# alexranaldi/CWSL_DIGI

Measured on AMD Instinct MI355X. Metric: IQ Msamples/s demod+sync per GPU; concurrent FT8 slots at real-time; % HBM roofline, higher is better.
Workload: dtype f32

## Files before the change

### cwsl_digi_amd/csrc/sync_kernels.hpp

```cpp
#pragma once
#include <hip/hip_runtime.h>
#include <stdint.h>

namespace cwslg {

constexpr int FT8_NSPS = 1920, FT8_NSTEP = 480, FT8_NHSYM = 372, FT8_NH1 = 1920, FT8_JZ = 62, FT8_NMAX = 180000;
constexpr int FT4_NFFT1 = 2304, FT4_NSTEP = 576, FT4_NHSYM = 122, FT4_NH1 = 1152, FT4_NMAX = 72576;
constexpr int FT4_ROW = 1168;
constexpr int SYNC_BAND = 32;
constexpr int SYNC_MAXCAND_CAP = 600;
constexpr int SYNC_MAXPRE = 1000;

struct SyncConfig {
    bool enabled = false;
    float syncmin = 1.5f;
    float syncmin_ft4 = 1.2f;
    int max_cand = 200;
    int f_lo_hz = 200, f_hi_hz = 3000;
    int ia = 64, ib = 960, nbins = 976;
    struct Kept {
        bool ft4_coherent = true;
        int order = 0;
        bool ft4_soft = false;
        bool ft8_soft = false;
// ... 973 lines not shown
            for (int k = 0; k < 7; ++k) {
                const float2 v = *reinterpret_cast<const float2 *>(&s_s[rr + 2 * k][2 * mp]);
                acc.x = acc.x + v.x;
                acc.y = acc.y + v.y;
            }
            *reinterpret_cast<float2 *>(c0 + 2 * mp) = acc;
        }
        __builtin_amdgcn_fence(__ATOMIC_RELEASE, "wavefront");
        __builtin_amdgcn_wave_barrier();
        __builtin_amdgcn_fence(__ATOMIC_ACQUIRE, "wavefront");
        const int j = 2 * lane - FT8_JZ;
        const bool ok0 = j <= FT8_JZ, ok1 = j + 1 <= FT8_JZ;
        SyncPair sy = SyncPair{0.0f, 0.0f};
        if (ok0) sy = costas_sync2(s_s, c0, rr, j);
        const unsigned long long ka = ok0 ? sync_key(sy.a, j + FT8_JZ) : 0ull;
        const unsigned long long kb = ok1 ? sync_key(sy.b, j + 1 + FT8_JZ) : 0ull;
        unsigned long long k2 = (kb > ka) ? kb : ka;
        unsigned long long k1 = 0ull;
        if (ok0 && j >= -10 && j <= 10) k1 = ka;
        if (ok1 && j + 1 >= -10 && j + 1 <= 10 && kb > k1) k1 = kb;
        k2 = wave_max_u64(k2);
        k1 = wave_max_u64(k1);
        if (lane == 0) {
            w->red[bin] = key_value(k1);  w->jpeak[bin] = (255 - (int)(k1 & 0xFFu)) - FT8_JZ;
            w->red2[bin] = key_value(k2); w->jpeak2[bin] = (255 - (int)(k2 & 0xFFu)) - FT8_JZ;
        }
        __builtin_amdgcn_fence(__ATOMIC_RELEASE, "wavefront");
        __builtin_amdgcn_wave_barrier();
    }
}

#endif
constexpr int S2_PITCH = 378, S2_COL0 = 2;
constexpr int DPP_ROW_MIRROR = 0x140;

__device__ __forceinline__ float wave_max_f32(float v)
{
    v = fmaxf(v, dpp_get<DPP_XOR1>(v));
    v = fmaxf(v, dpp_get<DPP_XOR2>(v));
    v = fmaxf(v, dpp_get<DPP_HALF_MIRROR>(v));
    v = fmaxf(v, dpp_get<DPP_ROW_MIRROR>(v));
    const int vi = __float_as_int(v);
    const float r0 = __int_as_float(__builtin_amdgcn_readlane(vi, 0)), r1 = __int_as_float(__builtin_amdgcn_readlane(vi, 16));
    const float r2 = __int_as_float(__builtin_amdgcn_readlane(vi, 32)), r3 = __int_as_float(__builtin_amdgcn_readlane(vi, 48));
    return fmaxf(fmaxf(r0, r1), fmaxf(r2, r3));
}

__device__ __forceinline__ void wave_first_max(float v, int lag, float &best, int &best_lag)
{
    const float m = wave_max_f32(v);
    const unsigned long long hit = __builtin_amdgcn_ballot_w64(v == m);
    const int src = hit ? (int)__builtin_ctzll(hit) : 0;
    best = __int_as_float(__builtin_amdgcn_readlane(__float_as_int(v), src));
    best_lag = __builtin_amdgcn_readlane(lag, src);
}

#ifndef CWSLG_SEARCH_HOISTPTR
#define CWSLG_SEARCH_HOISTPTR 1
#endif
#ifndef CWSLG_SEARCH_DPPMAX
#define CWSLG_SEARCH_DPPMAX 1
#endif
__device__ __forceinline__ void wave_first_max2(float va, int laga, float vb, int lagb, float &besta, int &best_laga, float &bestb, int &best_lagb)
{
    float ma = va, mb = vb;
#define CWSLG_DPP_MAX2(CTRL)                                                                  \
    "v_max_f32_dpp %0, %0, %0 " CTRL "\n\t"                                                   \
    "v_max_f32_dpp %1, %1, %1 " CTRL "\n\t"                                                   \
    "s_nop 0\n\t"
    asm volatile("s_nop 1\n\t"
                 CWSLG_DPP_MAX2("quad_perm:[1,0,3,2] row_mask:0xf bank_mask:0xf")
                 CWSLG_DPP_MAX2("quad_perm:[2,3,0,1] row_mask:0xf bank_mask:0xf")
                 CWSLG_DPP_MAX2("row_half_mirror row_mask:0xf bank_mask:0xf")
                 CWSLG_DPP_MAX2("row_mirror row_mask:0xf bank_mask:0xf")
                 CWSLG_DPP_MAX2("row_bcast:15 row_mask:0xa bank_mask:0xf")
                 CWSLG_DPP_MAX2("row_bcast:31 row_mask:0xc bank_mask:0xf")
                 "s_nop 0"
                 : "+v"(ma), "+v"(mb));
#undef CWSLG_DPP_MAX2
    const float wa = __int_as_float(__builtin_amdgcn_readlane(__float_as_int(ma), 63));
    const float wb = __int_as_float(__builtin_amdgcn_readlane(__float_as_int(mb), 63));
    const unsigned long long hita = __builtin_amdgcn_ballot_w64(va == wa), hitb = __builtin_amdgcn_ballot_w64(vb == wb);
    const int srca = hita ? (int)__builtin_ctzll(hita) : 0, srcb = hitb ? (int)__builtin_ctzll(hitb) : 0;
    besta = __int_as_float(__builtin_amdgcn_readlane(__float_as_int(va), srca)); best_laga = __builtin_amdgcn_readlane(laga, srca);
    bestb = __int_as_float(__builtin_amdgcn_readlane(__float_as_int(vb), srcb)); best_lagb = __builtin_amdgcn_readlane(lagb, srcb);
}

__device__ __forceinline__ float div6_exact(float x)
{
    const float r = 0x1.555556p-3f;
    const float q0 = x * r;
    const float e = __builtin_fmaf(-6.0f, q0, x);
    float q = __builtin_fmaf(e, r, q0);
    if (__builtin_expect((__float_as_uint(x) & 0x7fffffffu) - 0x10000000u >= 0x6f800000u, 0)) q = x / 6.0f;
    return q;
}

__device__ __forceinline__ float sync_finish(float ta, float tb, float tc, float t0a, float t0b, float t0c)
{
    float t = ta + tb + tc;
    float t0 = t0a + t0b + t0c;
    t0 = div6_exact(t0 - t);
    const float sync_abc = t / t0;
    t = tb + tc;
    t0 = t0b + t0c;
    t0 = div6_exact(t0 - t);
    const float sync_bc = t / t0;
    float sy = (sync_abc > sync_bc) ? sync_abc : sync_bc;
    if (!(sy == sy)) sy = 0.0f;
    return sy;
}

__device__ __forceinline__ void sync_finish2(v2f ta, v2f tb, v2f tc, v2f ua, v2f ub, v2f uc, float &sx, float &sy)
{
    const float r = 0x1.555556p-3f;
    const float t1x = ta.x + tb.x + tc.x, t1y = ta.y + tb.y + tc.y;
    const float d1x = (ua.x + ub.x + uc.x) - t1x, d1y = (ua.y + ub.y + uc.y) - t1y;
    const float t2x = tb.x + tc.x, t2y = tb.y + tc.y;
    const float d2x = (ub.x + uc.x) - t2x, d2y = (ub.y + uc.y) - t2y;
    auto short6 = [&](float x) { const float q0 = x * r; return __builtin_fmaf(__builtin_fmaf(-6.0f, q0, x), r, q0); };
    auto biased = [](float x) { return (__float_as_uint(x) & 0x7fffffffu) - 0x10000000u; };
    float q1x = short6(d1x), q1y = short6(d1y), q2x = short6(d2x), q2y = short6(d2y);
    const unsigned worst = max(max(biased(d1x), biased(d1y)), max(biased(d2x), biased(d2y)));
    if (__builtin_expect(worst >= 0x6f800000u, 0)) { q1x = d1x / 6.0f; q1y = d1y / 6.0f; q2x = d2x / 6.0f; q2y = d2y / 6.0f; }
    const float ax = t1x / q1x, bx = t2x / q2x, ay = t1y / q1y, by = t2y / q2y;
    sx = (ax > bx) ? ax : bx;
    sy = (ay > by) ? ay : by;
    if (!(sx == sx)) sx = 0.0f;
    if (!(sy == sy)) sy = 0.0f;
}

#if defined(CWSLG_STAMP) && defined(CWSLG_STAMP_SYNC)
#define SSTAMP(slot)                                                                                \
    do {                                                                                            \
        const unsigned wg_ = blockIdx.y * gridDim.x + blockIdx.x;                                   \
        if (threadIdx.x == 0 && wg_ < 65536) {                                                      \
            unsigned long long t_;                                                                  \
            asm volatile("s_waitcnt vmcnt(0) lgkmcnt(0)\n\ts_memtime %0\n\ts_waitcnt lgkmcnt(0)" : "=s"(t_)::"memory");              \
            g_stamps[8 * wg_ + (slot)] = t_;                                                        \
        }                                                                                           \
    } while (0)
#define SSTAMP1(slot)                                                                               \
    do {                                                                                            \
        const unsigned wg_ = blockIdx.y * gridDim.x + blockIdx.x;                                   \
        if (threadIdx.x == 0 && wg_ < 65536) {                                                      \
            unsigned long long t_;                                                                  \
            asm volatile("s_waitcnt lgkmcnt(0)\n\ts_memtime %0\n\ts_waitcnt lgkmcnt(0)" : "=s"(t_)::"memory");              \
            g_stamps[8 * wg_ + (slot)] = t_;                                                        \
        }                                                                                           \
    } while (0)
#else
#define SSTAMP(slot) do { } while (0)
#define SSTAMP1(slot) do { } while (0)
#endif
#if CWSLG_LAB
__global__ __launch_bounds__(SYNC2D_NT, 4) void ft8_sync2d_v2_kernel(const SyncWork *__restrict__ works, int ia, int ib, int nbins)
{
    constexpr int ROWS = SYNC_BAND + 12, NW = SYNC2D_NT / 64;
    constexpr int UN = (FT8_NHSYM + NW - 1) / NW;
    __shared__ __attribute__((aligned(16))) float s_s[ROWS][S2_PITCH];
    __shared__ __attribute__((aligned(16))) float s_c0[NW][S2_PITCH];
    const SyncWork *w = works + blockIdx.y;
    const int tid = threadIdx.x, lane = tid & 63, wv = tid >> 6;
    const int i0 = ia + blockIdx.x * SYNC_BAND;
    {
        const CWSLG_GLOBAL float *sp = as_global(w->spectra) + i0 + lane;
        const bool on = lane < ROWS && i0 + lane < nbins;
        float v[UN];
#pragma unroll
        for (int q = 0; q < UN; ++q) {
            const int m = wv + NW * q;
            v[q] = (on && m < FT8_NHSYM) ? sp[(size_t)m * nbins] : 0.0f;
        }
        float *dst = &s_s[lane < ROWS ? lane : 0][S2_COL0 + 1 + wv];
#pragma unroll
        for (int q = 0; q < UN; ++q)
            if (lane < ROWS && wv + NW * q < FT8_NHSYM) dst[NW * q] = v[q];
        if (tid < ROWS) {
            float *row = s_s[tid];
            row[0] = 0.0f; row[1] = 0.0f; row[2] = 0.0f;
            row[S2_COL0 + 373] = 0.0f; row[S2_COL0 + 374] = 0.0f; row[S2_COL0 + 375] = 0.0f;
        }
    }
    __syncthreads();
    float *c0 = s_c0[wv];
    const int icos[7] = {3, 1, 4, 0, 6, 5, 2};
    const int j = 2 * lane - FT8_JZ;
    const bool ok0 = j <= FT8_JZ, ok1 = j + 1 <= FT8_JZ;
    const bool near0 = j >= -10 && j <= 10, near1 = j + 1 >= -10 && j + 1 <= 10;
    const float ninf = -__builtin_huge_valf();
    const int pa0 = lane - 24, pb0 = pa0 + 72, pc0 = pa0 + 144;
    constexpr int PP = S2_PITCH / 2;
    const v2f *s_s2 = reinterpret_cast<const v2f *>(&s_s[0][0]);
    v2f *c02 = reinterpret_cast<v2f *>(c0);
    {
        for (int rr = wv; rr < SYNC_BAND; rr += NW) {
            const int bin = i0 + rr;
            if (bin > ib) break;
            for (int mp = lane; mp < PP; mp += 64) {
                v2f acc = {0.0f, 0.0f};
#pragma unroll
                for (int k = 0; k < 7; ++k) acc = acc + s_s2[(rr + 2 * k) * PP + mp];
                c02[mp] = acc;
            }
            __builtin_amdgcn_fence(__ATOMIC_RELEASE, "wavefront");
            __builtin_amdgcn_wave_barrier();
            __builtin_amdgcn_fence(__ATOMIC_ACQUIRE, "wavefront");
            v2f ta = {0, 0}, tb = {0, 0}, tc = {0, 0}, ua = {0, 0}, ub = {0, 0}, uc = {0, 0};
#pragma unroll
            for (int n = 0; n < 7; ++n) {
                const v2f *row = s_s2 + (rr + 2 * icos[n]) * PP;
                int pa = pa0 + 2 * n; pa = pa < 0 ? 0 : pa;
                int pc = pc0 + 2 * n; pc = pc > PP - 1 ? PP - 1 : pc;
                const int pb = pb0 + 2 * n;
                const v2f va = row[pa], wa = c02[pa];
                const v2f vb = row[pb], wb = c02[pb];
                const v2f vc = row[pc], wc = c02[pc];
                ta = ta + va; ua = ua + wa;
                tb = tb + vb; ub = ub + wb;
                tc = tc + vc; uc = uc + wc;
            }
            const float sa = ok0 ? sync_finish(ta.x, tb.x, tc.x, ua.x, ub.x, uc.x) : ninf;
            const float sb = ok1 ? sync_finish(ta.y, tb.y, tc.y, ua.y, ub.y, uc.y) : ninf;
            const bool b2 = sb > sa;
            float r2; int l2;
            wave_first_max(b2 ? sb : sa, b2 ? j + 1 : j, r2, l2);
            const float na = near0 ? sa : ninf, nb = near1 ? sb : ninf;
            const bool b1 = nb > na;
            float r1; int l1;
            wave_first_max(b1 ? nb : na, b1 ? j + 1 : j, r1, l1);
            if (lane == 0) {
                as_global_rw(w->red)[bin] = r1;  as_global_rw(w->jpeak)[bin] = l1;
                as_global_rw(w->red2)[bin] = r2; as_global_rw(w->jpeak2)[bin] = l2;
            }
            __builtin_amdgcn_fence(__ATOMIC_RELEASE, "wavefront");
            __builtin_amdgcn_wave_barrier();
        }
    }
}

#endif
#include "sync2d_asm.inc"
template <int NW>
__device__ __forceinline__ void sync2d_search_band(const SyncWork *w, unsigned s_base, unsigned sC, int wvu, int lane, int i0, int ia, int ib)
{
    constexpr int PP = S2_PITCH / 2, RB = S2_PITCH * 4;
    static_assert(S2_PITCH == 378, "sync2d_asm.inc is generated for this row pitch");
    const int j = 2 * lane - FT8_JZ;
    const bool ok0 = j <= FT8_JZ, ok1 = j + 1 <= FT8_JZ;
    const bool near0 = j >= -10 && j <= 10, near1 = j + 1 >= -10 && j + 1 <= 10;
    const float ninf = -__builtin_huge_valf();
    unsigned vA[7], vC[3];
#pragma unroll
    for (int n = 0; n < 7; ++n) { const int p = lane - 24 + 2 * n; vA[n] = 8u * (unsigned)(p < 0 ? 0 : p); }
#pragma unroll
    for (int n = 4; n < 7; ++n) { const int p = lane + 120 + 2 * n; vC[n - 4] = 8u * (unsigned)(p > PP - 1 ? PP - 1 : p); }
    const unsigned vU = 8u * (unsigned)lane, vL2 = 8u * (unsigned)(lane + 128 > PP - 1 ? PP - 1 : lane + 128);
#if CWSLG_SEARCH_HOISTPTR
    float *const p_red = w->red, *const p_red2 = w->red2;
    int *const p_jpeak = w->jpeak, *const p_jpeak2 = w->jpeak2;
#endif
    int rr = wvu;
    while (rr < SYNC_BAND && i0 + rr < ia) rr += NW;
    bool live = rr < SYNC_BAND && i0 + rr <= ib;
    if (live) {
        const unsigned sN = (unsigned)__builtin_amdgcn_readfirstlane((int)(s_base + (unsigned)rr * RB));
        asm volatile(SYNC2D_ASM_C0_ONLY : : [vU] "v"(vU), [vL2] "v"(vL2), [sC] "s"(sC), [sN] "s"(sN) : SYNC2D_ASM_CLOBBERS);
    }
    SSTAMP(2);
    const int rr0 = rr;
    while (live) {
        const int bin = i0 + rr;
        const int rn = rr + NW;
        const bool more = rn < SYNC_BAND && i0 + rn <= ib;
        const unsigned sS = (unsigned)__builtin_amdgcn_readfirstlane((int)(s_base + (unsigned)rr * RB));
        const unsigned sN = sS + NW * RB;
        v2f ta, tb, tc, ua, ub, uc;
        if (more)
            asm volatile(SYNC2D_ASM_SEARCH_NEXT
                         : [ta] "=&v"(ta), [ua] "=&v"(ua), [tb] "=&v"(tb), [ub] "=&v"(ub), [tc] "=&v"(tc), [uc] "=&v"(uc)
                         : [vA0] "v"(vA[0]), [vA1] "v"(vA[1]), [vA2] "v"(vA[2]), [vA3] "v"(vA[3]), [vA4] "v"(vA[4]), [vA5] "v"(vA[5]), [vA6] "v"(vA[6]),
                           [vC4] "v"(vC[0]), [vC5] "v"(vC[1]), [vC6] "v"(vC[2]), [vU] "v"(vU), [vL2] "v"(vL2), [sS] "s"(sS), [sC] "s"(sC), [sN] "s"(sN)
                         : SYNC2D_ASM_CLOBBERS);
        else
            asm volatile(SYNC2D_ASM_SEARCH_LAST
                         : [ta] "=&v"(ta), [ua] "=&v"(ua), [tb] "=&v"(tb), [ub] "=&v"(ub), [tc] "=&v"(tc), [uc] "=&v"(uc)
                         : [vA0] "v"(vA[0]), [vA1] "v"(vA[1]), [vA2] "v"(vA[2]), [vA3] "v"(vA[3]), [vA4] "v"(vA[4]), [vA5] "v"(vA[5]), [vA6] "v"(vA[6]),
                           [vC4] "v"(vC[0]), [vC5] "v"(vC[1]), [vC6] "v"(vC[2]), [vU] "v"(vU), [sS] "s"(sS), [sC] "s"(sC)
                         : SYNC2D_ASM_CLOBBERS);
        if (rr == rr0) SSTAMP(3);
        float sa, sb;
#if CWSLG_SEARCH_DPPMAX
        sync_finish2(ta, tb, tc, ua, ub, uc, sa, sb);
#else
        sa = sync_finish(ta.x, tb.x, tc.x, ua.x, ub.x, uc.x);
        sb = sync_finish(ta.y, tb.y, tc.y, ua.y, ub.y, uc.y);
#endif
        asm volatile("" : "+v"(sa), "+v"(sb));
        sa = ok0 ? sa : ninf;
        sb = ok1 ? sb : ninf;
        if (rr == rr0) SSTAMP(4);
        const bool b2 = sb > sa;
        const float na = near0 ? sa : ninf, nb = near1 ? sb : ninf;
        const bool b1 = nb > na;
        float r1, r2; int l1, l2;
#if CWSLG_SEARCH_DPPMAX
        wave_first_max2(b2 ? sb : sa, b2 ? j + 1 : j, b1 ? nb : na, b1 ? j + 1 : j, r2, l2, r1, l1);
#else
        wave_first_max(b2 ? sb : sa, b2 ? j + 1 : j, r2, l2);
        wave_first_max(b1 ? nb : na, b1 ? j + 1 : j, r1, l1);
#endif
        if (lane == 0) {
#if CWSLG_SEARCH_HOISTPTR
            as_global_rw(p_red)[bin] = r1;  as_global_rw(p_jpeak)[bin] = l1;
            as_global_rw(p_red2)[bin] = r2; as_global_rw(p_jpeak2)[bin] = l2;
#else
            as_global_rw(w->red)[bin] = r1;  as_global_rw(w->jpeak)[bin] = l1;
            as_global_rw(w->red2)[bin] = r2; as_global_rw(w->jpeak2)[bin] = l2;
#endif
        }
        if (rr == rr0) SSTAMP(5);
        rr = rn;
        live = more;
    }
}

__global__ __launch_bounds__(SYNC2D_NT, 4) void ft8_sync2d_v3_kernel(const SyncWork *__restrict__ works, int ia, int ib, int nbins)
{
    constexpr int ROWS = SYNC_BAND + 12, NW = SYNC2D_NT / 64;
    constexpr int UN = (FT8_NHSYM + NW - 1) / NW;
    __shared__ __attribute__((aligned(16))) float s_s[ROWS][S2_PITCH];
    __shared__ __attribute__((aligned(16))) float s_c0[NW][S2_PITCH];
    const SyncWork *w = works + blockIdx.y;
    const int tid = threadIdx.x, lane = tid & 63, wv = tid >> 6;
    const int i0 = ia + blockIdx.x * SYNC_BAND;
    SSTAMP(0);
    {
        const CWSLG_GLOBAL float *sp = as_global(w->spectra) + i0 + lane;
        const bool on = lane < ROWS && i0 + lane < nbins;
        float v[UN];
#pragma unroll
        for (int q = 0; q < UN; ++q) {
            const int m = wv + NW * q;
            v[q] = (on && m < FT8_NHSYM) ? plane_load1(sp + (size_t)m * nbins) : 0.0f;
        }
        float *dst = &s_s[lane < ROWS ? lane : 0][S2_COL0 + 1 + wv];
#pragma unroll
        for (int q = 0; q < UN; ++q)
            if (lane < ROWS && wv + NW * q < FT8_NHSYM) dst[NW * q] = v[q];
        if (tid < ROWS) {
            float *row = s_s[tid];
            row[0] = 0.0f; row[1] = 0.0f; row[2] = 0.0f;
            row[S2_COL0 + 373] = 0.0f; row[S2_COL0 + 374] = 0.0f; row[S2_COL0 + 375] = 0.0f;
        }
    }
    __syncthreads();
    SSTAMP(1);
    const int wvu = __builtin_amdgcn_readfirstlane(wv);
    const unsigned s_base = (unsigned)(uintptr_t)&s_s[0][0];
    const unsigned sC = (unsigned)__builtin_amdgcn_readfirstlane((int)((unsigned)(uintptr_t)&s_c0[0][0] + (unsigned)wvu * (S2_PITCH * 4)));
#ifdef CWSLG_SYNC_STAGGER
    if (wvu >= NW / 2) __builtin_amdgcn_s_sleep(CWSLG_SYNC_STAGGER);
#endif
    sync2d_search_band<NW>(w, s_base, sC, wvu, lane, i0, ia, ib);
    SSTAMP(6);
}

__device__ __forceinline__ bool key_less(float va, int ia_, float vb, int ib_)
{
    if (va < vb) return true;
    if (va > vb) return false;
    return ia_ < ib_;
}

template <int NT>
__device__ void bitonic_sort_n(float *kv, int *ki, int n, int tid)
{
    for (int size = 2; size <= n; size <<= 1) {
        for (int stride = size >> 1; stride >= 1; stride >>= 1) {
            for (int t = tid; t < n / 2; t += NT) {
                const int lo = 2 * t - (t & (stride - 1));
                const int hi = lo + stride;
                const bool up = (lo & size) == 0;
                const float a = kv[lo], b = kv[hi];
                const int ai = ki[lo], bi = ki[hi];
                const bool sw = up ? key_less(b, bi, a, ai) : key_less(a, ai, b, bi);
                if (sw) { kv[lo] = b; kv[hi] = a; ki[lo] = bi; ki[hi] = ai; }
            }
            __syncthreads();
        }
    }
}

template <int NT>
struct CandLds {
    static constexpr size_t kv = 0, ki = kv + 2048 * 4, red = ki + 2048 * 4, red2 = red + (FT8_NH1 + 1) * 4 + 12, jp = red2 + (FT8_NH1 + 1) * 4 + 12,
                            jp2 = jp + (FT8_NH1 + 1) * 2 + 14, first = jp2 + (FT8_NH1 + 1) * 2 + 14, second = first + (FT8_NH1 + 2) * 2 + 12,
                            desc = second + (FT8_NH1 + 2) * 2 + 12, scan = desc + SYNC_MAXPRE * 4, scan_lo = scan + NT * 4, cbin = scan_lo + 1024 * 4,
                            clag = cbin + SYNC_MAXPRE * 4, csync = clag + SYNC_MAXPRE * 4, cf = csync + SYNC_MAXPRE * 4, ct = cf + SYNC_MAXPRE * 4,
                            base = ct + SYNC_MAXPRE * 4, n = base + 16, bytes = n + 16;
};

template <int NT>
__device__ void ft8_candidates_body(const SyncWork *w, int ia, int ib, float syncmin, int maxcand, int order, char *lds)
{
    using L = CandLds<NT>;
    float *s_kv = reinterpret_cast<float *>(lds + L::kv);
    int *s_ki = reinterpret_cast<int *>(lds + L::ki);
    float *s_red = reinterpret_cast<float *>(lds + L::red), *s_red2 = reinterpret_cast<float *>(lds + L::red2);
    short *s_jp = reinterpret_cast<short *>(lds + L::jp), *s_jp2 = reinterpret_cast<short *>(lds + L::jp2);
    short *s_first = reinterpret_cast<short *>(lds + L::first), *s_second = reinterpret_cast<short *>(lds + L::second);
    int *s_desc = reinterpret_cast<int *>(lds + L::desc);
    int *s_scan = reinterpret_cast<int *>(lds + L::scan);
    unsigned *s_scan_lo = reinterpret_cast<unsigned *>(lds + L::scan_lo);
    int *s_cbin = reinterpret_cast<int *>(lds + L::cbin), *s_clag = reinterpret_cast<int *>(lds + L::clag);
    float *s_csync = reinterpret_cast<float *>(lds + L::csync), *s_cf = reinterpret_cast<float *>(lds + L::cf), *s_ct = reinterpret_cast<float *>(lds + L::ct);
    float *s_base = reinterpret_cast<float *>(lds + L::base);
    int &s_n = *reinterpret_cast<int *>(lds + L::n);
    const int tid = threadIdx.x;
    const int iz = ib - ia + 1;
    const float df = 12000.0f / 3840.0f, tstep = 480.0f / 12000.0f;
    for (int i = ia + tid; i <= ib; i += NT) {
        s_red[i] = as_global(w->red)[i]; s_red2[i] = as_global(w->red2)[i]; s_jp[i] = (short)as_global(w->jpeak)[i]; s_jp2[i] = (short)as_global(w->jpeak2)[i];
    }
    for (int i = tid; i < FT8_NH1 + 2; i += NT) { s_first[i] = -1; s_second[i] = -1; }
    const int npct = (int)lroundf(0.40f * (float)iz);
    const int lim = min(SYNC_MAXPRE, iz);
    const int nsort = (iz <= 1024) ? 1024 : 2048;
    __syncthreads();
    for (int k = tid; k < nsort; k += NT) { s_kv[k] = (k < iz) ? s_red2[ia + k] : __builtin_huge_valf(); s_ki[k] = (k < iz) ? ia + k : 0x7fffffff; }
    __syncthreads();
    bitonic_sort_n<NT>(s_kv, s_ki, nsort, tid);
    if (tid == 0 && npct >= 1) s_base[1] = s_red2[s_ki[npct - 1]];
    __syncthreads();
    for (int k = tid; k < nsort; k += NT) { s_kv[k] = (k < iz) ? s_red[ia + k] : __builtin_huge_valf(); s_ki[k] = (k < iz) ? ia + k : 0x7fffffff; }
    __syncthreads();
    bitonic_sort_n<NT>(s_kv, s_ki, nsort, tid);
    if (tid == 0 && npct >= 1) s_base[0] = s_red[s_ki[npct - 1]];
    for (int r = tid; r < lim; r += NT) s_desc[r] = s_ki[iz - 1 - r];
    __syncthreads();
    if (npct < 1) { if (tid == 0) *as_global_rw(w->ncand) = 0; return; }
    const float base = s_base[0], base2 = s_base[1];
    for (int i = ia + tid; i <= ib; i += NT) { s_red[i] = s_red[i] / base; s_red2[i] = s_red2[i] / base2; }
    __syncthreads();
    constexpr int PER = (SYNC_MAXPRE + NT - 1) / NT;
    int cnt[PER], flags[PER];
    int local = 0;
#pragma unroll
    for (int q = 0; q < PER; ++q) {
        const int r = tid * PER + q;
        int f = 0;
        if (r < lim) {
            const int n = s_desc[r];
            if (s_red[n] >= syncmin) f |= 1;
            if (s_jp2[n] != s_jp[n] && s_red2[n] >= syncmin) f |= 2;
        }
        flags[q] = f;
        cnt[q] = (f & 1) + ((f >> 1) & 1);
        local += cnt[q];
    }
    s_scan[tid] = local;
    __syncthreads();
    for (int off = 1; off < NT; off <<= 1) {
        const int v = (tid >= off) ? s_scan[tid - off] : 0;
        __syncthreads();
        s_scan[tid] += v;
        __syncthreads();
    }
    int pos = s_scan[tid] - local;
#pragma unroll
    for (int q = 0; q < PER; ++q) {
        const int r = tid * PER + q;
        if (r < lim) {
            const int n = s_desc[r];
            if ((flags[q] & 1) && pos < SYNC_MAXPRE) { s_cbin[pos] = n; s_clag[pos] = s_jp[n]; s_csync[pos] = s_red[n]; s_first[n] = (short)pos; }
            if (flags[q] & 1) ++pos;
            if ((flags[q] & 2) && pos < SYNC_MAXPRE) { s_cbin[pos] = n; s_clag[pos] = s_jp2[n]; s_csync[pos] = s_red2[n]; s_second[n] = (short)pos; }
            if (flags[q] & 2) ++pos;
        }
    }
    if (tid == NT - 1) s_n = min(s_scan[NT - 1], SYNC_MAXPRE);
    __syncthreads();
    const int ncand = s_n;
    for (int i = tid; i < ncand; i += NT) { s_cf[i] = (float)s_cbin[i] * df; s_ct[i] = ((float)s_clag[i] - 0.5f) * tstep; }
    __syncthreads();
    short *s_done = reinterpret_cast<short *>(s_ki);
    short *s_ready = s_done + SYNC_MAXPRE;
    for (int i = tid; i < ncand; i += NT) s_done[i] = 0;
    __syncthreads();
    for (int round = 0; round <= ncand; ++round) {
        int pending = 0;
        for (int i = tid; i < ncand; i += NT) {
            if (s_done[i]) { s_ready[i] = 0; continue; }
            const int n = s_cbin[i];
            bool ok = true;
#pragma unroll
            for (int dn = -2; dn <= 2; ++dn) {
                const int nb = n + dn;
                if (nb < 0 || nb > FT8_NH1) continue;
                const int a = s_first[nb], b = s_second[nb];
                if (a >= 0 && a < i && !s_done[a]) ok = false;
                if (b >= 0 && b < i && !s_done[b]) ok = false;
            }
            s_ready[i] = ok ? 1 : 0;
            pending = 1;
        }
        if (!__syncthreads_or(pending)) break;
        for (int i = tid; i < ncand; i += NT) {
            if (!s_ready[i]) continue;
            const int n = s_cbin[i];
            int part[6];
            int np = 0;
#pragma unroll
            for (int dn = -1; dn <= 1; ++dn) {
                const int nb = n + dn;
                if (nb < 0 || nb > FT8_NH1) continue;
                const int a = s_first[nb], b = s_second[nb];
                if (a >= 0 && a < i) part[np++] = a;
                if (b >= 0 && b < i) part[np++] = b;
            }
#pragma unroll
            for (int x = 1; x < 6; ++x) {
                if (x < np) {
                    const int v = part[x];
                    int y = x - 1;
                    while (y >= 0 && part[y] > v) { part[y + 1] = part[y]; --y; }
                    part[y + 1] = v;
                }
            }
            const float fi = fabsf(s_cf[i]), ti = s_ct[i];
            float si = s_csync[i];
            for (int x = 0; x < np; ++x) {
                const int j = part[x];
                const float fdiff = fi - fabsf(s_cf[j]);
                const float tdiff = fabsf(ti - s_ct[j]);
                if (fabsf(fdiff) < 4.0f && tdiff < 0.04f) {
                    const float sj = s_csync[j];
                    if (si >= sj) s_csync[j] = 0.0f;
                    if (si < sj) si = 0.0f;
                }
            }
            s_csync[i] = si;
            s_done[i] = 1;
        }
        __syncthreads();
    }
    __syncthreads();
    unsigned *s_hi = reinterpret_cast<unsigned *>(s_kv);
    unsigned *s_lo = reinterpret_cast<unsigned *>(s_scan_lo);
    for (int i = tid; i < 1024; i += NT) {
        unsigned hi = 0xFFFFFFFFu, lo = 0xFFFFFFFFu;
        if (i < ncand && s_csync[i] >= syncmin) {
            unsigned u = __float_as_uint(s_csync[i]);
            u = (u & 0x80000000u) ? ~u : (u | 0x80000000u);
            hi = ~u;
            lo = ((unsigned)s_cbin[i] << 20) | ((unsigned)(s_clag[i] + FT8_JZ) << 12) | (unsigned)i;
            if (order) { hi = (unsigned)s_cbin[i]; lo = (unsigned)i; }
        }
        s_hi[i] = hi; s_lo[i] = lo;
    }
    __syncthreads();
    for (int size = 2; size <= 1024; size <<= 1) {
        for (int stride = size >> 1; stride >= 1; stride >>= 1) {
            for (int t = tid; t < 512; t += NT) {
                const int l0 = 2 * t - (t & (stride - 1));
                const int h0 = l0 + stride;
                const bool up = (l0 & size) == 0;
                const unsigned long long ka = ((unsigned long long)s_hi[l0] << 32) | s_lo[l0];
                const unsigned long long kb = ((unsigned long long)s_hi[h0] << 32) | s_lo[h0];
                const bool sw = up ? (kb < ka) : (ka < kb);
                if (sw) { s_hi[l0] = (unsigned)(kb >> 32); s_lo[l0] = (unsigned)kb; s_hi[h0] = (unsigned)(ka >> 32); s_lo[h0] = (unsigned)ka; }
            }
            __syncthreads();
        }
    }
    int nout = 0;
    for (int r = tid; r < 1024; r += NT) {
        if (s_hi[r] == 0xFFFFFFFFu && s_lo[r] == 0xFFFFFFFFu) continue;
        ++nout;
        if (r < maxcand) {
            const int i = (int)(s_lo[r] & 0xFFFu);
            CWSLG_GLOBAL SyncChannelBuffers::Cand *c = as_global_rw(w->cand) + r;
            c->freq_bin = s_cbin[i]; c->time_step = s_clag[i]; c->sync = s_csync[i]; c->freq_hz = s_cf[i]; c->dt_s = s_ct[i];
        }
    }
    if (tid == 0) s_n = 0;
    __syncthreads();
    if (nout) atomicAdd(&s_n, nout);
    __syncthreads();
    if (tid == 0) *as_global_rw(w->ncand) = min(s_n, maxcand);
}

template <int NT>
__global__ __launch_bounds__(NT) void ft8_candidates_kernel(const SyncWork *__restrict__ works, int ia, int ib,
                                                              float syncmin, int maxcand, int order)
{
    __shared__ __attribute__((aligned(16))) char s_pool[CandLds<NT>::bytes];
    ft8_candidates_body<NT>(works + blockIdx.x, ia, ib, syncmin, maxcand, order, s_pool);
}

constexpr int SYNCC_NT = 512;
__global__ __launch_bounds__(SYNCC_NT, 4) void ft8_sync_chan_kernel(const SyncWork *__restrict__ works, int ia, int ib, int nbins,
                                                                     float syncmin, int maxcand, int order)
{
    constexpr int ROWS = SYNC_BAND + 12, NW = SYNCC_NT / 64;
    constexpr int UN = (FT8_NHSYM + NW - 1) / NW;
    constexpr int PF = (FT8_NHSYM + 8 * NW - 1) / (8 * NW);
    constexpr size_t IMG_BYTES = (size_t)(ROWS + NW) * S2_PITCH * sizeof(float);
    constexpr size_t POOL_BYTES = IMG_BYTES > CandLds<SYNCC_NT>::bytes ? IMG_BYTES : CandLds<SYNCC_NT>::bytes;
    __shared__ __attribute__((aligned(16))) char s_pool[POOL_BYTES];
    float (*s_s)[S2_PITCH] = reinterpret_cast<float (*)[S2_PITCH]>(s_pool);
    float (*s_c0)[S2_PITCH] = reinterpret_cast<float (*)[S2_PITCH]>(s_pool + (size_t)ROWS * S2_PITCH * sizeof(float));
    const SyncWork *w = works + blockIdx.x;
    const int tid = threadIdx.x, lane = tid & 63, wv = tid >> 6;
    const int i_first = ia - (((ia - 20) % 32) + 32) % 32;
    const int nbands = (ib - i_first) / SYNC_BAND + 1;
    const CWSLG_GLOBAL float *spec = as_global(w->spectra);
    {
        const int col = i_first + lane;
        const bool on = lane < ROWS && col >= 0 && col < nbins;
        const CWSLG_GLOBAL float *sp = spec + (on ? col : 0);
        float v[UN];
#pragma unroll
        for (int q = 0; q < UN; ++q) {
            const int m = wv + NW * q;
            v[q] = (on && m < FT8_NHSYM) ? plane_load1(sp + (size_t)m * nbins) : 0.0f;
        }
        float *dst = &s_s[lane < ROWS ? lane : 0][S2_COL0 + 1 + wv];
#pragma unroll
        for (int q = 0; q < UN; ++q)
            if (lane < ROWS && wv + NW * q < FT8_NHSYM) dst[NW * q] = v[q];
        if (tid < ROWS) {
            float *row = s_s[tid];
            row[0] = 0.0f; row[1] = 0.0f; row[2] = 0.0f;
            row[S2_COL0 + 373] = 0.0f; row[S2_COL0 + 374] = 0.0f; row[S2_COL0 + 375] = 0.0f;
        }
    }
    __syncthreads();
    const int wvu = __builtin_amdgcn_readfirstlane(wv);
    const unsigned s_base = (unsigned)(uintptr_t)&s_s[0][0];
    const unsigned sC = (unsigned)__builtin_amdgcn_readfirstlane((int)((unsigned)(uintptr_t)&s_c0[0][0] + (unsigned)wvu * (S2_PITCH * 4)));
    const int s8 = lane >> 3, g4 = 4 * (lane & 7);
    for (int band = 0; band < nbands; ++band) {
        const int i0 = i_first + band * SYNC_BAND;
        v4f pf[PF];
        const bool more = band + 1 < nbands;
        if (band == 1) SSTAMP(0);
        if (more) {
            const int col = i0 + ROWS + g4;
            const bool on = col < nbins;
            const unsigned o0 = (unsigned)((on ? col : 0) + (8 * wv + s8) * nbins);
            const unsigned ostep = (unsigned)(8 * NW * nbins);
#pragma unroll
            for (int q = 0; q < PF; ++q) {
                const int m = 8 * (wv + NW * q) + s8;
                pf[q] = (on && m < FT8_NHSYM) ? plane_load4(reinterpret_cast<const CWSLG_GLOBAL v4f *>(spec + o0 + (unsigned)q * ostep)) : v4f{0.f, 0.f, 0.f, 0.f};
            }
        }
        if (band == 1) SSTAMP1(1);
        sync2d_search_band<NW>(w, s_base, sC, wvu, lane, i0, ia, ib);
        if (band == 1) SSTAMP1(6);
        if (!more) break;
        constexpr int NMV = 12 * S2_PITCH / 4, MVT = (NMV + SYNCC_NT - 1) / SYNCC_NT;
        static_assert((12 * S2_PITCH) % 4 == 0 && (SYNC_BAND * S2_PITCH) % 4 == 0, "16-byte moves");
        v4f mv[MVT];
#pragma unroll
        for (int q = 0; q < MVT; ++q) {
            const int e = tid + SYNCC_NT * q;
            mv[q] = (e < NMV) ? reinterpret_cast<const v4f *>(&s_s[SYNC_BAND][0])[e] : v4f{0.f, 0.f, 0.f, 0.f};
        }
        __syncthreads();
#pragma unroll
        for (int q = 0; q < MVT; ++q) {
            const int e = tid + SYNCC_NT * q;
            if (e < NMV) reinterpret_cast<v4f *>(&s_s[0][0])[e] = mv[q];
        }
        {
#pragma unroll
            for (int q = 0; q < PF; ++q) {
                const int m = 8 * (wv + NW * q) + s8;
                if (m < FT8_NHSYM) {
#pragma unroll
                    for (int e = 0; e < 4; ++e) s_s[12 + g4 + e][S2_COL0 + 1 + m] = pf[q][e];
                }
            }
        }
        __syncthreads();
        if (band == 1) SSTAMP(7);
    }
    __syncthreads();
    ft8_candidates_body<SYNCC_NT>(w, ia, ib, syncmin, maxcand, order, s_pool);
}

__device__ __forceinline__ double log10_fixed(double x)
{
    if (!(x > 0.0)) return -1.0e300;
    int e = 0;
    double m = x;
    while (m >= 1.4142135623730951) { m = m * 0.5; ++e; }
    while (m < 0.7071067811865476) { m = m * 2.0; --e; }
    const double t = (m - 1.0) / (m + 1.0), t2 = t * t;
    double s = 0.0;
    for (int k = 21; k >= 1; k -= 2) s = s * t2 + 1.0 / (double)k;
    const double ln_m = 2.0 * t * s;
    return ((double)e * 0.6931471805599453 + ln_m) * 0.4342944819032518;
}
__device__ __forceinline__ double exp10_fixed(double y)
{
    const double z = y * 3.321928094887362;
    double fl = (double)(long long)z;
    if (fl > z) fl = fl - 1.0;
    const double f = (z - fl) * 0.6931471805599453;
    double s = 1.0;
    for (int k = 22; k >= 1; --k) s = 1.0 + s * f / (double)k;
    long long n = (long long)fl;
    double p = 1.0;
    if (n >= 0) { for (long long q = 0; q < n && q < 2000; ++q) p = p * 2.0; }
    else { for (long long q = 0; q < -n && q < 2000; ++q) p = p * 0.5; }
    return s * p;
}

__global__ __launch_bounds__(256) void ft4_candidates_kernel(const SyncWork *__restrict__ works, int nfa, int nfb,
                                                              float syncmin, int maxcand, int order)
{
    constexpr int NB1 = FT4_NH1 + 1;
    __shared__ float s_savg[NB1], s_savsm[NB1], s_sdb[NB1], s_sbase[NB1];
    __shared__ float s_segbase[10];
    __shared__ double s_a[5];
    __shared__ double s_A[5][6];
    __shared__ int s_scan[256];
    __shared__ int s_ok;
    __shared__ int s_cbin[SYNC_MAXCAND_CAP];
    __shared__ float s_cs[SYNC_MAXCAND_CAP], s_cf[SYNC_MAXCAND_CAP];
    __shared__ unsigned s_hi[1024], s_lo[1024];
    const SyncWork *w = works + blockIdx.x;
    const int tid = threadIdx.x;
    const CWSLG_GLOBAL float *sp = as_global(w->spectra);
    CWSLG_GLOBAL int *ncand_out = as_global_rw(w->ncand);
    const float df = 12000.0f / (float)FT4_NFFT1;
    for (int i = tid; i < NB1; i += 256) {
        float acc = 0.0f;
        if (i >= 1) {
            for (int j = 0; j < FT4_NHSYM; ++j) acc = acc + sp[(size_t)j * FT4_ROW + i];
            acc = acc / (float)FT4_NHSYM;
        }
        s_savg[i] = acc; s_sbase[i] = 0.0f; s_sdb[i] = 0.0f;
    }
    if (tid == 0) s_ok = 1;
    __syncthreads();
    for (int i = tid; i < NB1; i += 256) {
        float t = 0.0f;
        if (i >= 8 && i <= FT4_NH1 - 7) {
#pragma unroll
            for (int q = -7; q <= 7; ++q) t = t + s_savg[i + q];
            t = t / 15.0f;
        }
        s_savsm[i] = t;
    }
    const int ia = nfa, ib = min(nfb, FT4_NH1);
    const int nseg = 10;
    const int nlen = (ib - ia + 1) / nseg, i0 = (ib - ia + 1) / 2;
    const double half = (double)(ib - ia + 1) / 2.0;
    const bool range_ok = (nfb - nfa) >= 20;
    if (!range_ok) { if (tid == 0) *ncand_out = 0; return; }
    for (int i = ia + tid; i <= ib; i += 256) s_sdb[i] = (float)(10.0 * log10_fixed((double)s_savg[i]));
    __syncthreads();
    {
        int jp = (int)lroundf(((float)nlen * 0.01f) * 10.0f);
        if (jp < 1) jp = 1;
        if (jp > nlen) jp = nlen;
        for (int e = tid; e < nseg * nlen; e += 256) {
            const int seg = e / nlen, q = e - seg * nlen;
            const int ja = ia + seg * nlen;
            const float v = s_sdb[ja + q];
            int less = 0, eq = 0;
            for (int x = 0; x < nlen; ++x) {
                const float o = s_sdb[ja + x];
                less += (o < v) ? 1 : 0;
                eq += (o == v) ? 1 : 0;
            }
            if (less <= jp - 1 && jp - 1 < less + eq) s_segbase[seg] = v;
        }
    }
    __syncthreads();
    if (tid == 0) {
        double S[9], Tm[5];
        for (int q = 0; q < 9; ++q) S[q] = 0.0;
        for (int q = 0; q < 5; ++q) Tm[q] = 0.0;
        int kz = 0;
        for (int n = 0; n < nseg; ++n) {
            const int ja = ia + n * nlen, jb = ja + nlen - 1;
            const float base = s_segbase[n];
            for (int i = ja; i <= jb; ++i) {
                if (s_sdb[i] <= base && kz < 1000) {
                    ++kz;
                    const double u = (double)(i - i0) / half, y = (double)s_sdb[i];
                    double p = 1.0;
                    for (int q = 0; q < 9; ++q) { S[q] = S[q] + p; if (q < 5) Tm[q] = Tm[q] + y * p; p = p * u; }
                }
            }
        }
        int ok = kz >= 5;
        double (&A)[5][6] = s_A;
        for (int r = 0; r < 5; ++r) { for (int cc = 0; cc < 5; ++cc) A[r][cc] = S[r + cc]; A[r][5] = Tm[r]; }
        for (int col = 0; col < 5 && ok; ++col) {
            int piv = col;
            for (int r = col + 1; r < 5; ++r) if (fabs(A[r][col]) > fabs(A[piv][col])) piv = r;
            if (A[piv][col] == 0.0) { ok = 0; break; }
            if (piv != col) for (int cc = 0; cc < 6; ++cc) { const double t = A[col][cc]; A[col][cc] = A[piv][cc]; A[piv][cc] = t; }
            for (int r = col + 1; r < 5; ++r) {
                const double f = A[r][col] / A[col][col];
                for (int cc = col; cc < 6; ++cc) A[r][cc] = A[r][cc] - f * A[col][cc];
            }
        }
        double a[5] = {0, 0, 0, 0, 0};
        if (ok) {
            for (int r = 4; r >= 0; --r) {
                double t = A[r][5];
                for (int cc = r + 1; cc < 5; ++cc) t = t - A[r][cc] * a[cc];
                a[r] = t / A[r][r];
            }
        }
        for (int q = 0; q < 5; ++q) s_a[q] = a[q];
        s_ok = ok;
    }
    __syncthreads();
    if (!s_ok) { if (tid == 0) *ncand_out = 0; return; }
    int bad = 0;
    for (int i = ia + tid; i <= ib; i += 256) {
        const double u = (double)(i - i0) / half;
        const float db = (float)(s_a[0] + u * (s_a[1] + u * (s_a[2] + u * (s_a[3] + u * s_a[4]))) + 0.65);
        const float b = (float)exp10_fixed((double)db / 10.0);
        s_sbase[i] = b;
        if (!(b > 0.0f)) bad = 1;
    }
    if (__syncthreads_or(bad)) { if (tid == 0) *ncand_out = 0; return; }
    for (int i = nfa + tid; i <= nfb; i += 256) s_savsm[i] = s_savsm[i] / s_sbase[i];
    __syncthreads();
    {
        CWSLG_GLOBAL float *red = as_global_rw(w->red), *red2 = as_global_rw(w->red2);
        for (int i = tid; i < NB1; i += 256) { red[i] = s_savsm[i]; red2[i] = s_sbase[i]; }
// ... 81 lines not shown
```

Measured before the change: 302,200.

## Sort candidates in registers with DPP lane exchanges and wave-level scan

Replaces the LDS-based bitonic sorts (two red/red2 percentile sorts and the final candidate sort) with a register-resident bitonic network. Compares within a lane run in registers, cross-lane strides use DPP/permlane swaps, and only large strides go through double-buffered LDS with a barrier. The block-wide Hillis-Steele prefix scan becomes a DPP wave scan plus a per-wave combine. Together these cut the many __syncthreads and LDS round trips in candidate selection. The cost is higher register pressure, more template instantiation, and a final sort sized to the next power of two of the candidate count. Optional timestamp hooks are also added for profiling.

Result: no change. 303,900 (median of 6 runs) (+0.6%).

```diff
diff --git a/cwsl_digi_amd/csrc/sync_kernels.hpp b/cwsl_digi_amd/csrc/sync_kernels.hpp
--- a/cwsl_digi_amd/csrc/sync_kernels.hpp
+++ b/cwsl_digi_amd/csrc/sync_kernels.hpp
@@ -1149,6 +1149,15 @@
 #else
 #define SSTAMP(slot) do { } while (0)
 #define SSTAMP1(slot) do { } while (0)
+#endif
+#if defined(CWSLG_STAMP) && defined(CWSLG_STAMP_SYNC) && defined(CWSLG_STAMP_SEL)
+#define SELSTAMP(slot) SSTAMP(slot)
+#define BANDSTAMP(slot) do { } while (0)
+#define BANDSTAMP1(slot) do { } while (0)
+#else
+#define SELSTAMP(slot) do { } while (0)
+#define BANDSTAMP(slot) SSTAMP(slot)
+#define BANDSTAMP1(slot) SSTAMP1(slot)
 #endif
 #if CWSLG_LAB
 __global__ __launch_bounds__(SYNC2D_NT, 4) void ft8_sync2d_v2_kernel(const SyncWork *__restrict__ works, int ia, int ib, int nbins)
@@ -1370,23 +1379,102 @@
     return ia_ < ib_;
 }
 
-template <int NT>
-__device__ void bitonic_sort_n(float *kv, int *ki, int n, int tid)
-{
-    for (int size = 2; size <= n; size <<= 1) {
-        for (int stride = size >> 1; stride >= 1; stride >>= 1) {
-            for (int t = tid; t < n / 2; t += NT) {
-                const int lo = 2 * t - (t & (stride - 1));
-                const int hi = lo + stride;
-                const bool up = (lo & size) == 0;
-                const float a = kv[lo], b = kv[hi];
-                const int ai = ki[lo], bi = ki[hi];
-                const bool sw = up ? key_less(b, bi, a, ai) : key_less(a, ai, b, bi);
-                if (sw) { kv[lo] = b; kv[hi] = a; ki[lo] = bi; ki[hi] = ai; }
-            }
+struct SortKey { unsigned a, b; };
+struct FloatIndexLess {
+    static __device__ __forceinline__ bool either(SortKey p, SortKey k, bool first)
+    {
+        const float pv = __uint_as_float(p.a), kv = __uint_as_float(k.a);
+        const bool less_pk = (pv < kv) | (((int)p.b < (int)k.b) & !(pv > kv));
+        return less_pk == first;
+    }
+};
+struct WordPairLess {
+    static __device__ __forceinline__ bool either(SortKey p, SortKey k, bool first)
+    {
+        const unsigned long long pk = ((unsigned long long)p.a << 32) | p.b, kk = ((unsigned long long)k.a << 32) | k.b;
+        return (pk < kk) == first;
+    }
+};
+struct SortBufs {
+    char *base;
+    unsigned off0, off1;
+    int flip;
+};
+template <int M>
+__device__ __forceinline__ unsigned lane_xor(unsigned v)
+{
+    static_assert(M == 1 || M == 2 || M == 4 || M == 8 || M == 16 || M == 32, "one bit of the lane number");
+    if constexpr (M == 1) return (unsigned)__builtin_amdgcn_update_dpp((int)v, (int)v, 0xB1, 0xf, 0xf, false);
+    else if constexpr (M == 2) return (unsigned)__builtin_amdgcn_update_dpp((int)v, (int)v, 0x4E, 0xf, 0xf, false);
+    else if constexpr (M == 8) return (unsigned)__builtin_amdgcn_update_dpp((int)v, (int)v, 0x128, 0xf, 0xf, false);
+    else if constexpr (M == 4) {
+        const int t = __builtin_amdgcn_update_dpp((int)v, (int)v, 0x104, 0xf, 0x5, false);
+        return (unsigned)__builtin_amdgcn_update_dpp(t, (int)v, 0x114, 0xf, 0xa, false);
+    } else if constexpr (M == 16) {
+        const auto s = __builtin_amdgcn_permlane16_swap(v, v, false, false);
+        return (__lane_id() & 16) ? s[0] : s[1];
+    } else {
+        const auto s = __builtin_amdgcn_permlane32_swap(v, v, false, false);
+        return (__lane_id() & 32) ? s[0] : s[1];
+    }
+}
+template <class LESS, int NT, int K, int SIZE, int STRIDE>
+__device__ __forceinline__ void sort_stage(SortKey (&k)[K], int tid, SortBufs &sb)
+{
+    if constexpr (STRIDE < K) {
+#pragma unroll
+        for (int r = 0; r < K; ++r) {
+            if (r & STRIDE) continue;
+            const bool up = ((tid * K + r) & SIZE) == 0;
+            const SortKey a = k[r], b = k[r + STRIDE];
+            const bool sw = LESS::either(b, a, up);
+            k[r].a = sw ? b.a : a.a; k[r].b = sw ? b.b : a.b;
+            k[r + STRIDE].a = sw ? a.a : b.a; k[r + STRIDE].b = sw ? a.b : b.b;
+        }
+    } else {
+        SortKey p[K];
+        if constexpr (STRIDE / K < 64) {
+#pragma unroll
+            for (int r = 0; r < K; ++r) { p[r].a = lane_xor<STRIDE / K>(k[r].a); p[r].b = lane_xor<STRIDE / K>(k[r].b); }
+        } else {
+            unsigned *pa = reinterpret_cast<unsigned *>(sb.base + (sb.flip ? sb.off1 : sb.off0)), *pb = pa + NT * K;
+            sb.flip ^= 1;
+#pragma unroll
+            for (int r = 0; r < K; ++r) { pa[tid * K + r] = k[r].a; pb[tid * K + r] = k[r].b; }
             __syncthreads();
-        }
-    }
+            const int j = (tid * K) ^ STRIDE;
+#pragma unroll
+            for (int r = 0; r < K; ++r) { p[r].a = pa[j + r]; p[r].b = pb[j + r]; }
+        }
+        const bool is_hi = ((tid * K) & STRIDE) != 0, up = ((tid * K) & SIZE) == 0;
+        const bool first = up != is_hi;
+#pragma unroll
+        for (int r = 0; r < K; ++r) {
+            const bool sw = LESS::either(p[r], k[r], first);
+            k[r].a = sw ? p[r].a : k[r].a; k[r].b = sw ? p[r].b : k[r].b;
+        }
+    }
+}
+template <class LESS, int NT, int K, int SIZE, int STRIDE>
+__device__ __forceinline__ void sort_strides(SortKey (&k)[K], int tid, SortBufs &sb)
+{
+    sort_stage<LESS, NT, K, SIZE, STRIDE>(k, tid, sb);
+    if constexpr (STRIDE > 1) sort_strides<LESS, NT, K, SIZE, STRIDE / 2>(k, tid, sb);
+}
+template <class LESS, int NT, int K, int SIZE = 2>
+__device__ __forceinline__ void sort_in_registers(SortKey (&k)[K], int n, int tid, SortBufs &sb)
+{
+    if (SIZE <= n) sort_strides<LESS, NT, K, SIZE, SIZE / 2>(k, tid, sb);
+    if constexpr (SIZE < NT * K) sort_in_registers<LESS, NT, K, 2 * SIZE>(k, n, tid, sb);
+}
+__device__ __forceinline__ int wave_scan_add(int x, int lane)
+{
+    x += __builtin_amdgcn_update_dpp(0, x, 0x111, 0xf, 0xf, false);
+    x += __builtin_amdgcn_update_dpp(0, x, 0x112, 0xf, 0xf, false);
+    x += __builtin_amdgcn_update_dpp(0, x, 0x114, 0xf, 0xf, false);
+    x += __builtin_amdgcn_update_dpp(0, x, 0x118, 0xf, 0xf, false);
+    const int r0 = __builtin_amdgcn_readlane(x, 15), r1 = __builtin_amdgcn_readlane(x, 31), r2 = __builtin_amdgcn_readlane(x, 47);
+    return x + (lane >= 16 ? r0 : 0) + (lane >= 32 ? r1 : 0) + (lane >= 48 ? r2 : 0);
 }
 
 template <int NT>
@@ -1398,18 +1486,45 @@
                             base = ct + SYNC_MAXPRE * 4, n = base + 16, bytes = n + 16;
 };
 
+template <int NT, int K>
+__device__ __forceinline__ void red_orders(char *lds, int ia, int iz, int npct, int lim, int tid)
+{
+    using L = CandLds<NT>;
+    static_assert(NT * K <= 2048 && 2 * (size_t)NT * K * 4 <= L::red - L::kv && 2 * (size_t)NT * K * 4 <= L::base - L::cbin, "the sorts' two LDS buffers");
+    int *s_desc = reinterpret_cast<int *>(lds + L::desc);
+    float *s_base = reinterpret_cast<float *>(lds + L::base);
+    SortBufs sb{lds, (unsigned)L::kv, (unsigned)L::cbin, 0};
+#pragma unroll 1
+    for (int pass = 0; pass < 2; ++pass) {
+        const float *src = reinterpret_cast<const float *>(lds + (pass ? L::red : L::red2));
+        SortKey k[K];
+#pragma unroll
+        for (int r = 0; r < K; ++r) {
+            const int p = tid * K + r;
+            k[r].a = __float_as_uint((p < iz) ? src[ia + p] : __builtin_huge_valf());
+            k[r].b = (p < iz) ? (unsigned)(ia + p) : 0x7fffffffu;
+        }
+        sort_in_registers<FloatIndexLess, NT, K>(k, NT * K, tid, sb);
+        SELSTAMP(2 + pass);
+#pragma unroll
+        for (int r = 0; r < K; ++r) {
+            const int p = tid * K + r;
+            if (p == npct - 1) s_base[1 - pass] = src[(int)k[r].b];
+            if (pass && p < iz && p >= iz - lim) s_desc[iz - 1 - p] = (int)k[r].b;
+        }
+    }
+}
+
 template <int NT>
-__device__ void ft8_candidates_body(const SyncWork *w, int ia, int ib, float syncmin, int maxcand, int order, char *lds)
+__device__ __forceinline__ void ft8_candidates_body(const SyncWork *w, int ia, int ib, float syncmin, int maxcand, int order, char *lds)
 {
     using L = CandLds<NT>;
-    float *s_kv = reinterpret_cast<float *>(lds + L::kv);
     int *s_ki = reinterpret_cast<int *>(lds + L::ki);
     float *s_red = reinterpret_cast<float *>(lds + L::red), *s_red2 = reinterpret_cast<float *>(lds + L::red2);
     short *s_jp = reinterpret_cast<short *>(lds + L::jp), *s_jp2 = reinterpret_cast<short *>(lds + L::jp2);
     short *s_first = reinterpret_cast<short *>(lds + L::first), *s_second = reinterpret_cast<short *>(lds + L::second);
     int *s_desc = reinterpret_cast<int *>(lds + L::desc);
     int *s_scan = reinterpret_cast<int *>(lds + L::scan);
-    unsigned *s_scan_lo = reinterpret_cast<unsigned *>(lds + L::scan_lo);
     int *s_cbin = reinterpret_cast<int *>(lds + L::cbin), *s_clag = reinterpret_cast<int *>(lds + L::clag);
     float *s_csync = reinterpret_cast<float *>(lds + L::csync), *s_cf = reinterpret_cast<float *>(lds + L::cf), *s_ct = reinterpret_cast<float *>(lds + L::ct);
     float *s_base = reinterpret_cast<float *>(lds + L::base);
@@ -1417,6 +1532,7 @@
     const int tid = threadIdx.x;
     const int iz = ib - ia + 1;
     const float df = 12000.0f / 3840.0f, tstep = 480.0f / 12000.0f;
+    SELSTAMP(1);
     for (int i = ia + tid; i <= ib; i += NT) {
         s_red[i] = as_global(w->red)[i]; s_red2[i] = as_global(w->red2)[i]; s_jp[i] = (short)as_global(w->jpeak)[i]; s_jp2[i] = (short)as_global(w->jpeak2)[i];
     }
@@ -1425,16 +1541,8 @@
     const int lim = min(SYNC_MAXPRE, iz);
     const int nsort = (iz <= 1024) ? 1024 : 2048;
     __syncthreads();
-    for (int k = tid; k < nsort; k += NT) { s_kv[k] = (k < iz) ? s_red2[ia + k] : __builtin_huge_valf(); s_ki[k] = (k < iz) ? ia + k : 0x7fffffff; }
-    __syncthreads();
-    bitonic_sort_n<NT>(s_kv, s_ki, nsort, tid);
-    if (tid == 0 && npct >= 1) s_base[1] = s_red2[s_ki[npct - 1]];
-    __syncthreads();
-    for (int k = tid; k < nsort; k += NT) { s_kv[k] = (k < iz) ? s_red[ia + k] : __builtin_huge_valf(); s_ki[k] = (k < iz) ? ia + k : 0x7fffffff; }
-    __syncthreads();
-    bitonic_sort_n<NT>(s_kv, s_ki, nsort, tid);
-    if (tid == 0 && npct >= 1) s_base[0] = s_red[s_ki[npct - 1]];
-    for (int r = tid; r < lim; r += NT) s_desc[r] = s_ki[iz - 1 - r];
+    if (nsort == 1024) red_orders<NT, 1024 / NT>(lds, ia, iz, npct, lim, tid);
+    else red_orders<NT, 2048 / NT>(lds, ia, iz, npct, lim, tid);
     __syncthreads();
     if (npct < 1) { if (tid == 0) *as_global_rw(w->ncand) = 0; return; }
     const float base = s_base[0], base2 = s_base[1];
@@ -1456,15 +1564,17 @@
         cnt[q] = (f & 1) + ((f >> 1) & 1);
         local += cnt[q];
     }
-    s_scan[tid] = local;
-    __syncthreads();
-    for (int off = 1; off < NT; off <<= 1) {
-        const int v = (tid >= off) ? s_scan[tid - off] : 0;
-        __syncthreads();
-        s_scan[tid] += v;
-        __syncthreads();
-    }
-    int pos = s_scan[tid] - local;
+    int incl = wave_scan_add(local, tid & 63);
+    if ((tid & 63) == 63) s_scan[tid >> 6] = incl;
+    __syncthreads();
+    int total = 0;
+#pragma unroll
+    for (int wv = 0; wv < NT / 64; ++wv) {
+        const int t = s_scan[wv];
+        if (wv < (tid >> 6)) incl += t;
+        total += t;
+    }
+    int pos = incl - local;
 #pragma unroll
     for (int q = 0; q < PER; ++q) {
         const int r = tid * PER + q;
@@ -1476,11 +1586,12 @@
             if (flags[q] & 2) ++pos;
         }
     }
-    if (tid == NT - 1) s_n = min(s_scan[NT - 1], SYNC_MAXPRE);
+    if (tid == 0) s_n = min(total, SYNC_MAXPRE);
     __syncthreads();
     const int ncand = s_n;
     for (int i = tid; i < ncand; i += NT) { s_cf[i] = (float)s_cbin[i] * df; s_ct[i] = ((float)s_clag[i] - 0.5f) * tstep; }
     __syncthreads();
+    SELSTAMP(4);
     short *s_done = reinterpret_cast<short *>(s_ki);
     short *s_ready = s_done + SYNC_MAXPRE;
     for (int i = tid; i < ncand; i += NT) s_done[i] = 0;
@@ -1543,9 +1654,13 @@
         __syncthreads();
     }
     __syncthreads();
-    unsigned *s_hi = reinterpret_cast<unsigned *>(s_kv);
-    unsigned *s_lo = reinterpret_cast<unsigned *>(s_scan_lo);
-    for (int i = tid; i < 1024; i += NT) {
+    SELSTAMP(5);
+    constexpr int KF = 1024 / NT;
+    static_assert(SYNC_MAXPRE <= 1024 && 2 * 1024 * 4 <= L::ki - L::kv && 2 * 1024 * 4 <= L::red - L::ki, "the final sort's two LDS buffers");
+    SortKey fk[KF];
+#pragma unroll
+    for (int q = 0; q < KF; ++q) {
+        const int i = tid * KF + q;
         unsigned hi = 0xFFFFFFFFu, lo = 0xFFFFFFFFu;
         if (i < ncand && s_csync[i] >= syncmin) {
             unsigned u = __float_as_uint(s_csync[i]);
@@ -1554,29 +1669,21 @@
             lo = ((unsigned)s_cbin[i] << 20) | ((unsigned)(s_clag[i] + FT8_JZ) << 12) | (unsigned)i;
             if (order) { hi = (unsigned)s_cbin[i]; lo = (unsigned)i; }
         }
-        s_hi[i] = hi; s_lo[i] = lo;
-    }
-    __syncthreads();
-    for (int size = 2; size <= 1024; size <<= 1) {
-        for (int stride = size >> 1; stride >= 1; stride >>= 1) {
-            for (int t = tid; t < 512; t += NT) {
-                const int l0 = 2 * t - (t & (stride - 1));
-                const int h0 = l0 + stride;
-                const bool up = (l0 & size) == 0;
-                const unsigned long long ka = ((unsigned long long)s_hi[l0] << 32) | s_lo[l0];
-                const unsigned long long kb = ((unsigned long long)s_hi[h0] << 32) | s_lo[h0];
-                const bool sw = up ? (kb < ka) : (ka < kb);
-                if (sw) { s_hi[l0] = (unsigned)(kb >> 32); s_lo[l0] = (unsigned)kb; s_hi[h0] = (unsigned)(ka >> 32); s_lo[h0] = (unsigned)ka; }
-            }
-            __syncthreads();
-        }
-    }
+        fk[q].a = hi; fk[q].b = lo;
+    }
+    int nfinal = 64;
+    while (nfinal < ncand) nfinal <<= 1;
+    SortBufs fsb{lds, (unsigned)L::kv, (unsigned)L::ki, 0};
+    sort_in_registers<WordPairLess, NT, KF>(fk, nfinal, tid, fsb);
+    SELSTAMP(6);
     int nout = 0;
-    for (int r = tid; r < 1024; r += NT) {
-        if (s_hi[r] == 0xFFFFFFFFu && s_lo[r] == 0xFFFFFFFFu) continue;
+#pragma unroll
+    for (int q = 0; q < KF; ++q) {
+        const int r = tid * KF + q;
+        if (fk[q].a == 0xFFFFFFFFu && fk[q].b == 0xFFFFFFFFu) continue;
         ++nout;
         if (r < maxcand) {
-            const int i = (int)(s_lo[r] & 0xFFFu);
+            const int i = (int)(fk[q].b & 0xFFFu);
             CWSLG_GLOBAL SyncChannelBuffers::Cand *c = as_global_rw(w->cand) + r;
             c->freq_bin = s_cbin[i]; c->time_step = s_clag[i]; c->sync = s_csync[i]; c->freq_hz = s_cf[i]; c->dt_s = s_ct[i];
         }
@@ -1586,6 +1693,7 @@
     if (nout) atomicAdd(&s_n, nout);
     __syncthreads();
     if (tid == 0) *as_global_rw(w->ncand) = min(s_n, maxcand);
+    SELSTAMP(7);
 }
 
 template <int NT>
@@ -1610,6 +1718,7 @@
     float (*s_c0)[S2_PITCH] = reinterpret_cast<float (*)[S2_PITCH]>(s_pool + (size_t)ROWS * S2_PITCH * sizeof(float));
     const SyncWork *w = works + blockIdx.x;
     const int tid = threadIdx.x, lane = tid & 63, wv = tid >> 6;
+    SELSTAMP(0);
     const int i_first = ia - (((ia - 20) % 32) + 32) % 32;
     const int nbands = (ib - i_first) / SYNC_BAND + 1;
     const CWSLG_GLOBAL float *spec = as_global(w->spectra);
@@ -1642,7 +1751,7 @@
         const int i0 = i_first + band * SYNC_BAND;
         v4f pf[PF];
         const bool more = band + 1 < nbands;
-        if (band == 1) SSTAMP(0);
+        if (band == 1) BANDSTAMP(0);
         if (more) {
             const int col = i0 + ROWS + g4;
             const bool on = col < nbins;
@@ -1654,9 +1763,9 @@
                 pf[q] = (on && m < FT8_NHSYM) ? plane_load4(reinterpret_cast<const CWSLG_GLOBAL v4f *>(spec + o0 + (unsigned)q * ostep)) : v4f{0.f, 0.f, 0.f, 0.f};
             }
         }
-        if (band == 1) SSTAMP1(1);
+        if (band == 1) BANDSTAMP1(1);
         sync2d_search_band<NW>(w, s_base, sC, wvu, lane, i0, ia, ib);
-        if (band == 1) SSTAMP1(6);
+        if (band == 1) BANDSTAMP1(6);
         if (!more) break;
         constexpr int NMV = 12 * S2_PITCH / 4, MVT = (NMV + SYNCC_NT - 1) / SYNCC_NT;
         static_assert((12 * S2_PITCH) % 4 == 0 && (SYNC_BAND * S2_PITCH) % 4 == 0, "16-byte moves");
@@ -1683,7 +1792,7 @@
             }
         }
         __syncthreads();
-        if (band == 1) SSTAMP(7);
+        if (band == 1) BANDSTAMP(7);
     }
     __syncthreads();
     ft8_candidates_body<SYNCC_NT>(w, ia, ib, syncmin, maxcand, order, s_pool);
```
